# DoHoonKim8/stark-verifier

Measured on AMD Instinct MI355X. Metric: recursive plonky2 proofs/sec (Semaphore d=20), higher is better.
Workload: dtype u64 (Goldilocks field, integer); 1 GPU; recursive: per unit one Semaphore signal (group 2^20, n=2^13, blowup 8, 28 FRI queries, 16 PoW bits, zk) + the recursive proof verifying it (n=2^14, same FRI parameters); 128 units per GPU per step, 10 prover contexts per GPU; all_gather of (nullifier|topic) + Poseidon aggregation root per step; parallelism=independent proofs sharded over ranks, no data-path collective, exchange=none (one rank): gl355_aggregation_root over the local leaves, units_proven_in_process=1674

## Files before the change

### include/gl355.h

```cpp
#ifndef GL355_H
#define GL355_H
#include <stddef.h>
#include <stdint.h>

#ifdef __cplusplus
extern "C" {
#endif

#define GL355_OK 0
#define GL355_E_INVALID_ARG (-1)
#define GL355_E_NO_DEVICE (-2)
#define GL355_E_OOM (-3)
#define GL355_E_HIP (-4)
#define GL355_E_UNSUPPORTED (-5)
#define GL355_E_WITNESS (-6)
#define GL355_E_VERIFY (-7)

#define GL355_P UINT64_C(0xFFFFFFFF00000001)
#define GL355_COSET_SHIFT UINT64_C(7)
#define GL355_SALT_SIZE 4
#define GL355_MAX_FRI_ARITY_BITS 4
#define GL355_MAX_UNITS 16

typedef struct gl355_ctx gl355_ctx;
// ... 354 lines not shown
int32_t gl355_plonk_vk_from_pk(const gl355_plonk_pk* pk, const uint64_t s_g2[16], gl355_plonk_vk** out);
int32_t gl355_plonk_vk_destroy(gl355_plonk_vk* vk);
int32_t gl355_plonk_verify(gl355_ctx* ctx , const gl355_plonk_vk* vk, const uint64_t* instances, const uint32_t* instance_lens,
                           const uint8_t* proof, uint64_t proof_len, int32_t* ok);
int32_t gl355_plonk_verify_batch(gl355_ctx* ctx , const gl355_plonk_vk* vk, uint32_t n_proofs, const uint64_t* instances ,
                                 const uint32_t* instance_lens , const uint8_t* const* proofs, const uint64_t* proof_lens,
                                 const uint8_t seed[32], int32_t* ok, int32_t* first_bad );
const char* gl355_plonk_verify_last_error(void);
int32_t gl355_plonk_verify_stage_ms(double ms[3]);
int32_t gl355_kzg_params_check(gl355_ctx* ctx, const uint64_t* g , uint64_t n_points, const uint64_t* g_lagrange ,
                               uint32_t log_n, const uint64_t s_g2[16], const uint8_t seed[32], int32_t* ok);

int32_t gl355_zs_partial_products(gl355_ctx* ctx, const uint64_t* wires, const uint64_t* sigmas,
                                  const uint64_t* k_is, uint32_t log_n, uint32_t n_routed,
                                  uint32_t max_degree, uint64_t beta, uint64_t gamma,
                                  uint64_t* z_out, uint64_t* pp_out);

enum { GL355_BN_M_MUL = 0, GL355_BN_M_ADD = 1, GL355_BN_M_SUB = 2, GL355_BN_M_CANON = 3, GL355_BN_M_FROM_INT = 4, GL355_BN_M_TO_INT = 5,
       GL355_BN_M_INV = 6, GL355_BN_M_IS_ZERO = 7, GL355_BN_M_EQ = 8, GL355_BN_FQ = 16,
       GL355_BN_F29_MUL = 32, GL355_BN_F29_MUL_FR = 33, GL355_BN_F29_ADD_NORM = 34, GL355_BN_F29_SUB_C2 = 35, GL355_BN_F29_SUB_C4 = 36,
       GL355_BN_F29_SUB_C8 = 37, GL355_BN_F29_SUB_C16 = 38, GL355_BN_F29_NEG_C2 = 39, GL355_BN_F29_FROM_U256 = 40, GL355_BN_F29_TO_U256 = 41,
       GL355_BN_F29_LIFT = 42, GL355_BN_F29_LIFT_INL = 43, GL355_BN_F29_LOWER = 44, GL355_BN_F29_IS_ZERO_MOD = 45, GL355_BN_F29_TABLE_FORM = 46,
       GL355_BN_F29_NORM = 47, GL355_BN_HASH_FR_ENTER = 48, GL355_BN_HASH_FR_LEAVE = 49 };
enum { GL355_BN_CHAIN_XYZZ = 0, GL355_BN_CHAIN_JAC29 = 1, GL355_BN_CHAIN_JAC = 2, GL355_BN_CHAIN_RED29_LIFT = 3, GL355_BN_CHAIN_RED29_RAW = 4,
       GL355_BN_CHAIN_J = 5 };
enum { GL355_BN_STEP_ADD = 0, GL355_BN_STEP_DOUBLE = 1, GL355_BN_STEP_ACC = 2, GL355_BN_STEP_SELF = 3, GL355_BN_STEP_MADD = 4 };
int32_t gl355_bn254_arith_batch(gl355_ctx* ctx, int32_t op, const uint32_t* a , const uint32_t* b , uint32_t* out ,
                                uint64_t n);
int32_t gl355_bn254_g1_chain(gl355_ctx* ctx, int32_t form, const uint32_t* operands , uint32_t n_operands,
                             const uint32_t* steps , uint32_t n_chains, uint32_t n_steps, uint32_t* trace );

enum { GL355_GL_MUL = 0, GL355_GL_MUL_MULTI1 = 1, GL355_GL_MUL_MULTI2 = 2, GL355_GL_MUL_MULTI3 = 3, GL355_GL_MUL_MULTI4 = 4, GL355_GL_MUL_FILL = 5,
       GL355_GL_MUL2_FILL = 6, GL355_GL_SQR = 7, GL355_GL_SBOX = 8, GL355_GL_SBOX4 = 9, GL355_GL_RECOMBINE = 10, GL355_GL_RECOMBINE_MULTI4 = 11,
       GL355_GL_PARTIAL_ROUNDS = 13 };
int32_t gl355_gl_arith_batch(gl355_ctx* ctx, int32_t op, const uint64_t* a , const uint64_t* b , uint64_t* out , uint64_t n);
int32_t gl355_poseidon_permute_lanes(gl355_ctx* ctx, int32_t form, uint64_t* states , uint64_t count);


int32_t gl355_bn254_g1_msm_bits(gl355_ctx* ctx, const uint64_t* points, const gl355_msm_bases* bases , const uint64_t* scalars, uint64_t n,
                                uint32_t n_sets, uint32_t max_bits, uint64_t* results , uint32_t plan_out[4] );
int32_t gl355_plonk_pk_commit_columns(gl355_plonk_pk* pk, uint32_t which, const uint64_t* columns , uint32_t sets, uint64_t tail,
                                      uint64_t* results );

#ifdef __cplusplus
}
#endif
#endif
```

### stark-verifier_amd/csrc/gl_field.cuh

```cuda
#pragma once
#include <hip/hip_runtime.h>
#include <stdint.h>

#define GL_P 0xFFFFFFFF00000001ull
#define GL_EPS 0xFFFFFFFFull

#define GL_DEV __device__ __forceinline__
#define GL_HD __host__ __device__ __forceinline__

#if defined(__HIP_DEVICE_COMPILE__)
#define GL_UNPRED(c) (c)
#else
#define GL_UNPRED(c) __builtin_unpredictable(c)
#endif

GL_HD uint64_t gl_canon(uint64_t a) { return a >= GL_P ? a - GL_P : a; }

GL_HD uint64_t gl_add(uint64_t a, uint64_t b) {
    uint64_t s = a + b;
    if (GL_UNPRED(s < a)) {
        s += GL_EPS;
        if (GL_UNPRED(s < GL_EPS)) s += GL_EPS;
    }
    return s;
}

GL_HD uint64_t gl_add_canonical(uint64_t a, uint64_t c) {
    uint64_t s = a + c;
    if (GL_UNPRED(s < a)) s += GL_EPS;
    return s;
}

GL_HD uint64_t gl_sub(uint64_t a, uint64_t b) {
    uint64_t d = a - b;
    if (GL_UNPRED(a < b)) {
        uint64_t e = d - GL_EPS;
        if (GL_UNPRED(d < GL_EPS)) e -= GL_EPS;
        d = e;
    }
    return d;
}

GL_HD uint64_t gl_neg(uint64_t a) { return gl_sub(0, a); }

#ifndef GL_MUL_VARIANT
#define GL_MUL_VARIANT 1
#endif
#if GL_MUL_VARIANT != 1 && GL_MUL_VARIANT != 2
#error "GL_MUL_VARIANT is 1 (carry steps in inline asm) or 2 (compiler-scheduled)"
#endif
#ifdef GL_EXPERIMENT_NO_HAZARD_NOP
#define GL_HAZARD_NOP ""
#else
#define GL_HAZARD_NOP "s_nop 1\n\t"
#endif
#if defined(__HIPCC__)
#if GL_MUL_VARIANT == 1
GL_DEV uint64_t gl_dev_sub32(uint32_t lo0, uint32_t lo1, uint32_t sub32) {
    uint32_t x0, x1, m;
    asm("v_sub_co_u32_e32 %0, vcc, %3, %5\n\t" GL_HAZARD_NOP ""
        "v_subbrev_co_u32_e32 %1, vcc, 0, %4, vcc\n\t" GL_HAZARD_NOP ""
        "v_cndmask_b32_e64 %2, 0, -1, vcc\n\t"
        "v_sub_co_u32_e32 %0, vcc, %0, %2\n\t" GL_HAZARD_NOP ""
        "v_subbrev_co_u32_e32 %1, vcc, 0, %1, vcc"
        : "=&v"(x0), "=&v"(x1), "=&v"(m) : "v"(lo0), "v"(lo1), "v"(sub32) : "vcc");
    return ((uint64_t)x1 << 32) | x0;
}
GL_DEV uint64_t gl_dev_add_mul_eps(uint64_t x, uint32_t k) {
    uint64_t r, carry;
    uint32_t m;
    asm("v_mad_u64_u32 %0, %1, %3, -1, %4\n\t" GL_HAZARD_NOP "v_cndmask_b32_e64 %2, 0, -1, %1"
        : "=v"(r), "=s"(carry), "=v"(m) : "v"(k), "v"(x));
    return r + (uint64_t)m;
}
GL_DEV uint64_t gl_dev_mid(uint32_t a1, uint32_t b0, uint64_t u, uint32_t* v0) {
    uint64_t v, carry;
    uint32_t ch;
    asm("v_mad_u64_u32 %0, %1, %3, %4, %5\n\t" GL_HAZARD_NOP "v_cndmask_b32_e64 %2, 0, 1, %1"
        : "=v"(v), "=s"(carry), "=v"(ch) : "v"(a1), "v"(b0), "v"(u));
    *v0 = (uint32_t)v;
    return ((uint64_t)ch << 32) | (v >> 32);
}
#else
GL_DEV uint64_t gl_dev_sub32(uint32_t lo0, uint32_t lo1, uint32_t sub32) {
    unsigned long x, y;
    const bool b = __builtin_usubl_overflow(((unsigned long)lo1 << 32) | lo0, (unsigned long)sub32, &x);
    __builtin_usubl_overflow(x, (unsigned long)(b ? 0xFFFFFFFFu : 0u), &y);
    return y;
}
GL_DEV uint64_t gl_dev_add_mul_eps(uint64_t x, uint32_t k) {
    const uint64_t r = (uint64_t)k * 0xFFFFFFFFu + x;
    return r + (r < x ? 0xFFFFFFFFu : 0u);
}
GL_DEV uint64_t gl_dev_mid(uint32_t a1, uint32_t b0, uint64_t u, uint32_t* v0) {
    const uint64_t v = (uint64_t)a1 * b0 + u;
    *v0 = (uint32_t)v;
    return ((uint64_t)(v < u ? 1u : 0u) << 32) | (v >> 32);
}
#endif
#endif

GL_HD uint64_t gl_reduce128(uint64_t lo, uint64_t hi) {
#if defined(__HIP_DEVICE_COMPILE__)
    return gl_dev_add_mul_eps(gl_dev_sub32((uint32_t)lo, (uint32_t)(lo >> 32), (uint32_t)(hi >> 32)), (uint32_t)hi);
#else
    uint32_t hi_hi = (uint32_t)(hi >> 32), hi_lo = (uint32_t)hi;
    uint64_t t0 = lo - hi_hi;
    if (GL_UNPRED(lo < hi_hi)) t0 -= GL_EPS;
    uint64_t t1 = ((uint64_t)hi_lo << 32) - hi_lo;
    uint64_t r = t0 + t1;
    if (GL_UNPRED(r < t1)) r += GL_EPS;
    return r;
#endif
}

GL_HD uint64_t gl_mul(uint64_t a, uint64_t b) {
#if defined(__HIP_DEVICE_COMPILE__)
    const uint32_t a0 = (uint32_t)a, a1 = (uint32_t)(a >> 32), b0 = (uint32_t)b, b1 = (uint32_t)(b >> 32);
    const uint64_t t = (uint64_t)a0 * b0;
    const uint64_t u = (uint64_t)a0 * b1 + (t >> 32);
    uint32_t v0;
    const uint64_t mid = gl_dev_mid(a1, b0, u, &v0);
    const uint64_t w = (uint64_t)a1 * b1 + mid;
    return gl_dev_add_mul_eps(gl_dev_sub32((uint32_t)t, v0, (uint32_t)(w >> 32)), (uint32_t)w);
#else
    unsigned __int128 pr = (unsigned __int128)a * b;
    return gl_reduce128((uint64_t)pr, (uint64_t)(pr >> 64));
#endif
}

GL_HD uint64_t gl_sqr(uint64_t a) { return gl_mul(a, a); }

#if defined(__HIPCC__) && GL_MUL_VARIANT == 1
template <int N>
GL_DEV void gl_mul_multi(const uint64_t (&a)[N], const uint64_t (&b)[N], uint64_t (&r)[N]) {
    static_assert(N >= 1 && N <= 4, "1 .. 4 products");
#define GL_MM_SB() __builtin_amdgcn_sched_barrier(0)
#define GL_MM_READ(INS, ...)                                               \
    do {                                                                   \
        if (N == 1) asm("s_nop 1\n\t" INS : __VA_ARGS__);                  \
        else if (N == 2 && j == 0) asm("s_nop 0\n\t" INS : __VA_ARGS__);   \
        else asm(INS : __VA_ARGS__);                                       \
    } while (0)
    uint32_t a0[N], a1[N], b0[N], b1[N], ch[N], x0[N], x1[N], m[N];
    uint64_t t[N], u[N], v[N], w[N], c[N];
#pragma unroll
    for (int j = 0; j < N; j++) { a0[j] = (uint32_t)a[j]; a1[j] = (uint32_t)(a[j] >> 32); b0[j] = (uint32_t)b[j]; b1[j] = (uint32_t)(b[j] >> 32); }
#pragma unroll
    for (int j = 0; j < N; j++) { t[j] = (uint64_t)a0[j] * b0[j]; u[j] = (uint64_t)a0[j] * b1[j] + (t[j] >> 32); }
    GL_MM_SB();
#pragma unroll
    for (int j = 0; j < N; j++) { asm("v_mad_u64_u32 %0, %1, %2, %3, %4" : "=v"(v[j]), "=s"(c[j]) : "v"(a1[j]), "v"(b0[j]), "v"(u[j])); GL_MM_SB(); }
#pragma unroll
    for (int j = 0; j < N; j++) { GL_MM_READ("v_cndmask_b32_e64 %0, 0, 1, %1", "=v"(ch[j]) : "s"(c[j])); GL_MM_SB(); }
#pragma unroll
    for (int j = 0; j < N; j++) w[j] = (uint64_t)a1[j] * b1[j] + (((uint64_t)ch[j] << 32) | (v[j] >> 32));
    GL_MM_SB();
#pragma unroll
    for (int j = 0; j < N; j++) { asm("v_sub_co_u32_e64 %0, %1, %2, %3" : "=v"(x0[j]), "=s"(c[j]) : "v"((uint32_t)t[j]), "v"((uint32_t)(w[j] >> 32))); GL_MM_SB(); }
#pragma unroll
    for (int j = 0; j < N; j++) { GL_MM_READ("v_subb_co_u32_e64 %0, %1, %2, 0, %1", "=v"(x1[j]), "+s"(c[j]) : "v"((uint32_t)v[j])); GL_MM_SB(); }
#pragma unroll
    for (int j = 0; j < N; j++) { GL_MM_READ("v_cndmask_b32_e64 %0, 0, -1, %1", "=v"(m[j]) : "s"(c[j])); GL_MM_SB(); }
#pragma unroll
    for (int j = 0; j < N; j++) { asm("v_sub_co_u32_e64 %0, %1, %0, %2" : "+v"(x0[j]), "=s"(c[j]) : "v"(m[j])); GL_MM_SB(); }
#pragma unroll
    for (int j = 0; j < N; j++) { GL_MM_READ("v_subb_co_u32_e64 %0, %1, %0, 0, %1", "+v"(x1[j]), "+s"(c[j])); GL_MM_SB(); }
#pragma unroll
    for (int j = 0; j < N; j++) {
        const uint64_t x = ((uint64_t)x1[j] << 32) | x0[j];
        asm("v_mad_u64_u32 %0, %1, %2, -1, %3" : "=v"(r[j]), "=s"(c[j]) : "v"((uint32_t)w[j]), "v"(x));
        GL_MM_SB();
    }
#pragma unroll
    for (int j = 0; j < N; j++) { GL_MM_READ("v_cndmask_b32_e64 %0, 0, 1, %1", "=v"(m[j]) : "s"(c[j])); GL_MM_SB(); }
#pragma unroll
    for (int j = 0; j < N; j++) asm("v_mad_u64_u32 %0, %1, %2, -1, %0" : "+v"(r[j]), "=s"(c[j]) : "v"(m[j]));
#undef GL_MM_READ
#undef GL_MM_SB
}
template <class F>
GL_DEV uint64_t gl_mul_fill(uint64_t a, uint64_t b, F&& fill) {
#define GL_MF_SB() __builtin_amdgcn_sched_barrier(0)
    const uint32_t a0 = (uint32_t)a, a1 = (uint32_t)(a >> 32), b0 = (uint32_t)b, b1 = (uint32_t)(b >> 32);
    const uint64_t t = (uint64_t)a0 * b0;
    const uint64_t u = (uint64_t)a0 * b1 + (t >> 32);
    uint64_t v, c, r;
    uint32_t ch, x0, x1, m;
    GL_MF_SB();
    asm("v_mad_u64_u32 %0, %1, %2, %3, %4" : "=v"(v), "=s"(c) : "v"(a1), "v"(b0), "v"(u)); GL_MF_SB();
    fill(0); GL_MF_SB();
    asm("v_cndmask_b32_e64 %0, 0, 1, %1" : "=v"(ch) : "s"(c)); GL_MF_SB();
    const uint64_t w = (uint64_t)a1 * b1 + (((uint64_t)ch << 32) | (v >> 32)); GL_MF_SB();
    asm("v_sub_co_u32_e64 %0, %1, %2, %3" : "=v"(x0), "=s"(c) : "v"((uint32_t)t), "v"((uint32_t)(w >> 32))); GL_MF_SB();
    fill(1); GL_MF_SB();
    asm("v_subb_co_u32_e64 %0, %1, %2, 0, %1" : "=v"(x1), "+s"(c) : "v"((uint32_t)v)); GL_MF_SB();
    fill(2); GL_MF_SB();
    asm("v_cndmask_b32_e64 %0, 0, -1, %1" : "=v"(m) : "s"(c)); GL_MF_SB();
    asm("v_sub_co_u32_e64 %0, %1, %0, %2" : "+v"(x0), "=s"(c) : "v"(m)); GL_MF_SB();
    fill(3); GL_MF_SB();
    asm("v_subb_co_u32_e64 %0, %1, %0, 0, %1" : "+v"(x1), "+s"(c)); GL_MF_SB();
    const uint64_t x = ((uint64_t)x1 << 32) | x0;
    asm("v_mad_u64_u32 %0, %1, %2, -1, %3" : "=v"(r), "=s"(c) : "v"((uint32_t)w), "v"(x)); GL_MF_SB();
    fill(4); GL_MF_SB();
    asm("v_cndmask_b32_e64 %0, 0, 1, %1" : "=v"(m) : "s"(c)); GL_MF_SB();
    asm("v_mad_u64_u32 %0, %1, %2, -1, %0" : "+v"(r), "=s"(c) : "v"(m));
    return r;
}
template <class F>
GL_DEV void gl_mul2_fill(const uint64_t (&a)[2], const uint64_t (&b)[2], uint64_t (&r)[2], F&& fill) {
// ... 148 lines not shown
```

### stark-verifier_amd/csrc/gl_hook.hip

```cpp
#include "gl355_internal.h"
#include "poseidon_lanes.cuh"

namespace gl355 {

static int hk_gl_width(int32_t op) {
    switch (op) {
    case GL355_GL_MUL: case GL355_GL_MUL_MULTI1: case GL355_GL_MUL_FILL: case GL355_GL_SQR: case GL355_GL_SBOX: case GL355_GL_RECOMBINE: return 1;
    case GL355_GL_MUL_MULTI2: case GL355_GL_MUL2_FILL: return 2;
    case GL355_GL_MUL_MULTI3: return 3;
    case GL355_GL_MUL_MULTI4: case GL355_GL_SBOX4: case GL355_GL_RECOMBINE_MULTI4: return 4;
    case GL355_GL_PARTIAL_ROUNDS: return 12;
    default: return 0;
    }
}

template <int N> GL_DEV void hk_mul_multi(const uint64_t* a, const uint64_t* b, uint64_t* out) {
    uint64_t x[N], y[N], r[N];
#pragma unroll
    for (int j = 0; j < N; j++) { x[j] = a[j]; y[j] = b[j]; }
    gl_mul_multi<N>(x, y, r);
#pragma unroll
    for (int j = 0; j < N; j++) out[j] = r[j];
}

struct HkRow {
    uint64_t xr[5], al, ah;
    GL_DEV HkRow(uint64_t a, uint64_t b) {
#pragma unroll
        for (int k = 0; k < 5; k++) xr[k] = a * (uint64_t)(k + 1) + b;
        al = (uint32_t)b; ah = b >> 32;
    }
    GL_DEV void term(int k) {
        al += (uint64_t)(uint32_t)xr[k] * PSD_CIRC_DEV[k];
        ah += (uint64_t)(uint32_t)(xr[k] >> 32) * PSD_CIRC_DEV[k];
    }
};

__global__ void __launch_bounds__(256) gl_arith_hook_kernel(int32_t op, int32_t width, const uint64_t* a, const uint64_t* b, uint64_t* out, uint64_t n) {
    const uint64_t i = (blockIdx.x * (uint64_t)blockDim.x + threadIdx.x) * (uint64_t)width;
    if (i >= n) return;
    const uint64_t* pa = a + i;
    const uint64_t* pb = b + i;
    uint64_t* po = out + i;
    switch (op) {
// ... 6 lines not shown
        HkRow row(pa[0], pb[0]);
        po[0] = gl_mul_fill(pa[0], pb[0], [&](int k) { row.term(k); });
        po[n] = row.al; po[2 * n] = row.ah;
        break;
    }
    case GL355_GL_MUL2_FILL: {
        HkRow row(pa[0], pb[0]);
        const uint64_t x[2] = {pa[0], pa[1]}, y[2] = {pb[0], pb[1]};
        uint64_t r[2];
        gl_mul2_fill(x, y, r, [&](int k) { row.term(k); });
        po[0] = r[0]; po[1] = r[1];
        po[n] = row.al; po[2 * n] = row.ah;
        po[n + 1] = 0; po[2 * n + 1] = 0;
        break;
    }
    case GL355_GL_SQR: po[0] = gl_sqr(pa[0]); break;
    case GL355_GL_SBOX: po[0] = psd_sbox(pa[0]); break;
    case GL355_GL_SBOX4: {
        uint64_t x0 = pa[0], x1 = pa[1], x2 = pa[2], x3 = pa[3];
        psd_sbox4(x0, x1, x2, x3);
        po[0] = x0; po[1] = x1; po[2] = x2; po[3] = x3;
        break;
    }
    case GL355_GL_RECOMBINE: po[0] = psd_recombine(pa[0], pb[0]); break;
    case GL355_GL_PARTIAL_ROUNDS: {
        uint64_t s[12];
#pragma unroll
        for (int j = 0; j < 12; j++) s[j] = pa[j];
        psd_partial_rounds_b3(s);
#pragma unroll
        for (int j = 0; j < 12; j++) po[j] = s[j];
        break;
    }
    default: {
        const uint64_t al[4] = {pa[0], pa[1], pa[2], pa[3]}, ah[4] = {pb[0], pb[1], pb[2], pb[3]};
        uint64_t r[4];
        psd_recombine_multi<4>(al, ah, r);
        po[0] = r[0]; po[1] = r[1]; po[2] = r[2]; po[3] = r[3];
        break;
    }
    }
}

template <int FORM>
__global__ void __launch_bounds__(64) poseidon_lanes_hook_kernel(uint64_t* states, uint64_t count) {
    __shared__ uint64_t rings[4][24];
    const int li = threadIdx.x & 15, grp = threadIdx.x >> 4;
    uint64_t g = blockIdx.x * 4ull + grp;
    const bool valid = g < count;
    if (!valid) g = 0;
    uint64_t s = (li < 12) ? states[g * 12 + li] : 0;
    s = psd_permute_lanes<FORM>(s, li, rings[grp]);
    if (valid && li < 12) states[g * 12 + li] = gl_canon(s);
}

}

using namespace gl355;

extern "C" {
int32_t gl355_gl_arith_batch(gl355_ctx* h, int32_t op, const uint64_t* a, const uint64_t* b, uint64_t* out, uint64_t n) {
    Ctx* ctx = ctx_of(h);
    if (!ctx) return GL355_E_INVALID_ARG;
    if (hipSetDevice(ctx->device) != hipSuccess) return ctx->fail(GL355_E_HIP, "hipSetDevice failed");
    const int width = hk_gl_width(op);
    if (!width) return ctx->fail(GL355_E_INVALID_ARG, "gl_arith_batch: bad op");
    if (n % (uint64_t)width) return ctx->fail(GL355_E_INVALID_ARG, "gl_arith_batch: n is not a multiple of the op's records per lane");
    if (n == 0) return GL355_OK;
    const bool two = !(op == GL355_GL_SQR || op == GL355_GL_SBOX || op == GL355_GL_SBOX4 || op == GL355_GL_PARTIAL_ROUNDS);
    if (!a || !out || (two && !b)) return ctx->fail(GL355_E_INVALID_ARG, "gl_arith_batch: null argument");
    const uint64_t lanes = n / (uint64_t)width;
    if ((lanes + 255) / 256 > 0x7FFFFFFFull) return ctx->fail(GL355_E_UNSUPPORTED, "gl_arith_batch: too many records");
    const uint64_t out_words = (op == GL355_GL_MUL_FILL || op == GL355_GL_MUL2_FILL) ? 3 * n : n;
    Staged sa(ctx), sb(ctx), so(ctx);
    GL355_TRY(sa.open(a, n * 8, 1));
    GL355_TRY(sb.open(two ? b : a, n * 8, 1));
    GL355_TRY(so.open(out, out_words * 8, 2));
    hipLaunchKernelGGL(gl_arith_hook_kernel, dim3((uint32_t)((lanes + 255) / 256)), dim3(256), 0, ctx->stream, op, (int32_t)width, sa.as<const uint64_t>(),
                       sb.as<const uint64_t>(), so.as<uint64_t>(), n);
    GL355_HIP(ctx, hipGetLastError());
    return so.finish();
}

int32_t gl355_poseidon_permute_lanes(gl355_ctx* h, int32_t form, uint64_t* states, uint64_t count) {
    Ctx* ctx = ctx_of(h);
    if (!ctx) return GL355_E_INVALID_ARG;
    if (hipSetDevice(ctx->device) != hipSuccess) return ctx->fail(GL355_E_HIP, "hipSetDevice failed");
    if (form != 0 && form != 3) return ctx->fail(GL355_E_INVALID_ARG, "poseidon_permute_lanes: form is 0 or 3");
    if (count == 0) return GL355_OK;
    if (!states) return ctx->fail(GL355_E_INVALID_ARG, "poseidon_permute_lanes: null states");
    if ((count + 3) / 4 > 0x7FFFFFFFull) return ctx->fail(GL355_E_UNSUPPORTED, "poseidon_permute_lanes: too many states");
    Staged s(ctx);
    GL355_TRY(s.open(states, count * 96, 3));
    const dim3 grid((uint32_t)((count + 3) / 4)), block(64);
    if (form == 3) hipLaunchKernelGGL(poseidon_lanes_hook_kernel<3>, grid, block, 0, ctx->stream, s.as<uint64_t>(), count);
    else hipLaunchKernelGGL(poseidon_lanes_hook_kernel<0>, grid, block, 0, ctx->stream, s.as<uint64_t>(), count);
    GL355_HIP(ctx, hipGetLastError());
    return s.finish();
}
}
```

### stark-verifier_amd/csrc/poseidon.cuh

```cuda
#pragma once
#include "gl_field.cuh"
#if GL_MUL_VARIANT != 1
#error "poseidon.cuh is written on the inline-asm product and its lock-step groups: GL_MUL_VARIANT 1"
#endif

#define PSD_TABLE_QUAL __device__ __constant__ const
#include "poseidon_tables.h"

namespace gl355 {

GL_DEV uint64_t psd_sbox(uint64_t x) {
    const uint64_t x2 = gl_sqr(x);
    const uint64_t a[2] = {x, x2}, b[2] = {x2, x2};
    uint64_t r[2];
    gl_mul_multi<2>(a, b, r);
    return gl_mul(r[0], r[1]);
}

GL_DEV uint64_t psd_recombine(uint64_t al, uint64_t ah) {
    uint32_t t1 = (uint32_t)(al >> 32), top;
    asm("v_add_co_u32_e32 %0, vcc, %0, %2\n\t" GL_HAZARD_NOP "v_addc_co_u32_e32 %1, vcc, 0, %3, vcc"
        : "+v"(t1), "=v"(top) : "v"((uint32_t)ah), "v"((uint32_t)(ah >> 32)) : "vcc");
    return gl_dev_add_mul_eps(((uint64_t)t1 << 32) | (uint32_t)al, top);
}

GL_DEV void psd_sbox4(uint64_t& x0, uint64_t& x1, uint64_t& x2, uint64_t& x3) {
    const uint64_t a[4] = {x0, x1, x2, x3};
    uint64_t sq[4], c3[4], c4[4], o[4];
    gl_mul_multi<4>(a, a, sq);
    gl_mul_multi<4>(a, sq, c3);
    gl_mul_multi<4>(sq, sq, c4);
    gl_mul_multi<4>(c3, c4, o);
    x0 = o[0]; x1 = o[1]; x2 = o[2]; x3 = o[3];
}
template <int N>
GL_DEV void psd_recombine_multi(const uint64_t (&al)[N], const uint64_t (&ah)[N], uint64_t (&out)[N]) {
    static_assert(N >= 3, "three or more: no wait states of their own");
    uint32_t t1[N], top[N], m[N];
    uint64_t c[N], r[N];
#pragma unroll
    for (int j = 0; j < N; j++) {
        asm("v_add_co_u32_e64 %0, %1, %2, %3" : "=v"(t1[j]), "=s"(c[j]) : "v"((uint32_t)(al[j] >> 32)), "v"((uint32_t)ah[j]));
        __builtin_amdgcn_sched_barrier(0);
    }
#pragma unroll
    for (int j = 0; j < N; j++) {
        asm("v_addc_co_u32_e64 %0, %1, 0, %2, %1" : "=v"(top[j]), "+s"(c[j]) : "v"((uint32_t)(ah[j] >> 32)));
        __builtin_amdgcn_sched_barrier(0);
    }
#pragma unroll
    for (int j = 0; j < N; j++) {
        const uint64_t x = ((uint64_t)t1[j] << 32) | (uint32_t)al[j];
        asm("v_mad_u64_u32 %0, %1, %2, -1, %3" : "=v"(r[j]), "=s"(c[j]) : "v"(top[j]), "v"(x));
        __builtin_amdgcn_sched_barrier(0);
    }
#pragma unroll
    for (int j = 0; j < N; j++) {
        asm("v_cndmask_b32_e64 %0, 0, -1, %1" : "=v"(m[j]) : "s"(c[j]));
        __builtin_amdgcn_sched_barrier(0);
    }
#pragma unroll
    for (int j = 0; j < N; j++) out[j] = r[j] + (uint64_t)m[j];
}

#define PSD_MDS_CHAIN(C0)                                                                                  \
    "v_mad_u64_u32 %0, %1, %2, " #C0 ", %14\n\tv_mad_u64_u32 %0, %1, %3, 15, %0\n\tv_mad_u64_u32 %0, %1, %4, 41, %0\n\t" \
    "v_mad_u64_u32 %0, %1, %5, 16, %0\n\tv_mad_u64_u32 %0, %1, %6, 2, %0\n\tv_mad_u64_u32 %0, %1, %7, 28, %0\n\t"      \
    "v_mad_u64_u32 %0, %1, %8, 13, %0\n\tv_mad_u64_u32 %0, %1, %9, 13, %0\n\tv_mad_u64_u32 %0, %1, %10, 39, %0\n\t"    \
    "v_mad_u64_u32 %0, %1, %11, 18, %0\n\tv_mad_u64_u32 %0, %1, %12, 34, %0\n\tv_mad_u64_u32 %0, %1, %13, 20, %0"
template <int R>
GL_DEV uint64_t psd_mds_chain(const uint32_t (&x)[12], uint64_t addend) {
    uint64_t acc, unused;
#define PSD_X(i) "v"(x[((i) + R) % 12])
    if constexpr (R == 0)
        asm(PSD_MDS_CHAIN(25) : "=&v"(acc), "=&s"(unused) : PSD_X(0), PSD_X(1), PSD_X(2), PSD_X(3), PSD_X(4), PSD_X(5), PSD_X(6),
            PSD_X(7), PSD_X(8), PSD_X(9), PSD_X(10), PSD_X(11), "s"(addend));
    else
        asm(PSD_MDS_CHAIN(17) : "=&v"(acc), "=&s"(unused) : PSD_X(0), PSD_X(1), PSD_X(2), PSD_X(3), PSD_X(4), PSD_X(5), PSD_X(6),
            PSD_X(7), PSD_X(8), PSD_X(9), PSD_X(10), PSD_X(11), "s"(addend));
#undef PSD_X
    return acc;
}
template <int R, class RC>
GL_DEV void psd_mds_rows(uint64_t (&s)[12], const uint32_t (&lo)[12], const uint32_t (&hi)[12], RC rc) {
    if constexpr (R < 12) {
        const uint64_t c0 = rc[R], c1 = rc[R + 1], c2 = rc[R + 2], c3 = rc[R + 3];
        const uint64_t al[4] = {psd_mds_chain<R>(lo, (uint32_t)c0), psd_mds_chain<R + 1>(lo, (uint32_t)c1), psd_mds_chain<R + 2>(lo, (uint32_t)c2),
                                psd_mds_chain<R + 3>(lo, (uint32_t)c3)};
        const uint64_t ah[4] = {psd_mds_chain<R>(hi, c0 >> 32), psd_mds_chain<R + 1>(hi, c1 >> 32), psd_mds_chain<R + 2>(hi, c2 >> 32),
                                psd_mds_chain<R + 3>(hi, c3 >> 32)};
        uint64_t o[4];
        __builtin_amdgcn_sched_barrier(0);
        psd_recombine_multi<4>(al, ah, o);
        s[R] = o[0]; s[R + 1] = o[1]; s[R + 2] = o[2]; s[R + 3] = o[3];
        psd_mds_rows<R + 4, RC>(s, lo, hi, rc);
    }
}
template <class RC>
GL_DEV void psd_mds(uint64_t (&s)[12], RC rc) {
    uint32_t lo[12], hi[12];
#pragma unroll
    for (int i = 0; i < 12; i++) { lo[i] = (uint32_t)s[i]; hi[i] = (uint32_t)(s[i] >> 32); }
    psd_mds_rows<0, RC>(s, lo, hi, rc);
}


#undef PSD_TABLE_QUAL
#define PSD_TABLE_QUAL __device__ __constant__
#include "poseidon_b3tables.h"

typedef const __attribute__((address_space(4))) uint32_t* psd_b3tab;
typedef const __attribute__((address_space(4))) uint64_t* psd_b3add;
GL_DEV void psd_b3_term(uint64_t& lo, uint64_t& hi, uint32_t c, uint64_t v) {
    uint64_t unused;
    asm("v_mad_u64_u32 %0, %2, %3, %4, %0\n\tv_mad_u64_u32 %1, %2, %3, %5, %1"
        : "+v"(lo), "+v"(hi), "=&s"(unused) : "s"(c), "v"((uint32_t)v), "v"((uint32_t)(v >> 32)));
}
GL_DEV void psd_b3_terms5(uint64_t& lo, uint64_t& hi, const uint32_t* c, const uint64_t* v) {
    uint64_t unused;
#define PSD_V(i) "v"((uint32_t)v[i]), "v"((uint32_t)(v[i] >> 32))
    asm("v_mad_u64_u32 %0, %2, %3, %8, %0\n\tv_mad_u64_u32 %1, %2, %3, %9, %1\n\t"
        "v_mad_u64_u32 %0, %2, %4, %10, %0\n\tv_mad_u64_u32 %1, %2, %4, %11, %1\n\t"
        "v_mad_u64_u32 %0, %2, %5, %12, %0\n\tv_mad_u64_u32 %1, %2, %5, %13, %1\n\t"
        "v_mad_u64_u32 %0, %2, %6, %14, %0\n\tv_mad_u64_u32 %1, %2, %6, %15, %1\n\t"
        "v_mad_u64_u32 %0, %2, %7, %16, %0\n\tv_mad_u64_u32 %1, %2, %7, %17, %1"
        : "+v"(lo), "+v"(hi), "=&s"(unused)
        : "s"(c[0]), "s"(c[1]), "s"(c[2]), "s"(c[3]), "s"(c[4]), PSD_V(0), PSD_V(1), PSD_V(2), PSD_V(3), PSD_V(4));
#undef PSD_V
}
GL_DEV void psd_b3_term_first(uint64_t& lo, uint64_t& hi, uint32_t c, uint64_t v, const uint64_t (&add)[2]) {
    uint64_t unused;
    asm("v_mov_b64 %0, %6\n\tv_mov_b64 %1, %7\n\t"
        "v_mad_u64_u32 %0, %2, %3, %4, %0\n\tv_mad_u64_u32 %1, %2, %3, %5, %1"
        : "=&v"(lo), "=&v"(hi), "=&s"(unused) : "s"(c), "v"((uint32_t)v), "v"((uint32_t)(v >> 32)), "s"(add[0]), "s"(add[1]));
}
struct PsdB3Row {
    uint32_t w[14];
    uint64_t a[2];
};
template <int NT>
GL_DEV void psd_b3_load(PsdB3Row& k, psd_b3tab c, psd_b3add add) {
#pragma unroll
    for (int i = 0; i < NT; i++) k.w[i] = c[i];
    k.a[0] = add[0]; k.a[1] = add[1];
}
template <int NX, int NT_NEXT>
GL_DEV void psd_b3_dot(const uint64_t (&u)[12], const uint64_t (&x)[3], PsdB3Row& k, psd_b3tab next, psd_b3add add_next, uint64_t& lo, uint64_t& hi) {
    const PsdB3Row cur = k;
    psd_b3_term_first(lo, hi, cur.w[0], u[1], cur.a);
    __builtin_amdgcn_sched_barrier(0);
    if constexpr (NT_NEXT > 0) psd_b3_load<NT_NEXT>(k, next, add_next);
    __builtin_amdgcn_sched_barrier(0);
    psd_b3_terms5(lo, hi, &cur.w[1], &u[2]);
    psd_b3_terms5(lo, hi, &cur.w[6], &u[7]);
#pragma unroll
    for (int t = 0; t < NX; t++) psd_b3_term(lo, hi, cur.w[11 + t], x[t]);
    __builtin_amdgcn_sched_barrier(0);
}
template <int R>
GL_DEV void psd_b3_out(uint64_t (&o)[12], const uint64_t (&u)[12], const uint64_t (&x)[3], psd_b3tab mac, psd_b3add add, PsdB3Row& k) {
    if constexpr (R < 12) {
        constexpr int W = PSD_B3_ROW_WORDS;
        uint64_t al[4], ah[4], r[4];
        psd_b3_dot<3, 14>(u, x, k, mac + W * (R + 3), add + 2 * (R + 3), al[0], ah[0]);
        psd_b3_dot<3, 14>(u, x, k, mac + W * (R + 4), add + 2 * (R + 4), al[1], ah[1]);
        psd_b3_dot<3, 14>(u, x, k, mac + W * (R + 5), add + 2 * (R + 5), al[2], ah[2]);
        psd_b3_dot<3, (R + 3 < 11 ? 14 : 0)>(u, x, k, mac + W * (R + 6), add + 2 * (R + 6), al[3], ah[3]);
        psd_recombine_multi<4>(al, ah, r);
        o[R] = r[0]; o[R + 1] = r[1]; o[R + 2] = r[2]; o[R + 3] = r[3];
        __builtin_amdgcn_sched_barrier(0);
        psd_b3_out<R + 4>(o, u, x, mac, add, k);
    }
}
GL_DEV void psd_partial_rounds_b3(uint64_t (&s)[12]) {
#pragma unroll 1
    for (int blk = 0; blk < PSD_B3_BLOCKS; blk++) {
        constexpr int W = PSD_B3_ROW_WORDS;
        psd_b3add add = (psd_b3add)PSD_B3_ADD + blk * 2 * 14;
        psd_b3tab mac = (psd_b3tab)PSD_B3_MAC;
        asm volatile("" : "+s"(mac), "+s"(add));
        PsdB3Row k;
        psd_b3_load<12>(k, mac, add);
        __builtin_amdgcn_sched_barrier(0);
        uint64_t x[3], o[12], lo, hi;
        x[0] = psd_sbox(s[0]);
        __builtin_amdgcn_sched_barrier(0);
        psd_b3_dot<1, 13>(s, x, k, mac + W, add + 2, lo, hi);
        x[1] = psd_sbox(psd_recombine(lo, hi));
        __builtin_amdgcn_sched_barrier(0);
        psd_b3_dot<2, 14>(s, x, k, mac + 2 * W, add + 4, lo, hi);
        x[2] = psd_sbox(psd_recombine(lo, hi));
        __builtin_amdgcn_sched_barrier(0);
        psd_b3_out<0>(o, s, x, mac, add, k);
#pragma unroll
        for (int i = 0; i < 12; i++) s[i] = o[i];
    }
    psd_b3add rc26 = (psd_b3add)PSD_ALL_RC + 12 * 26;
    asm volatile("" : "+s"(rc26));
    s[0] = psd_sbox(s[0]);
    psd_mds(s, rc26);
}

constexpr int psd_rounds_per_iter = 2;
GL_DEV void psd_dense_rounds(uint64_t (&s)[12], int r0, int r1) {
#pragma unroll 1
    for (int r = r0; r < r1; r += psd_rounds_per_iter) {
#pragma unroll
        for (int h = 0; h < psd_rounds_per_iter; h++) {
#pragma unroll
            for (int i = 0; i < 12; i += 4) psd_sbox4(s[i], s[i + 1], s[i + 2], s[i + 3]);
            psd_mds(s, &PSD_ALL_RC[12 * (r + h + 1)]);
        }
    }
}
GL_DEV void psd_permute(uint64_t (&s)[12]) {
#pragma unroll
    for (int i = 0; i < 12; i++) s[i] = gl_add_canonical(s[i], PSD_ALL_RC[i]);
    psd_dense_rounds(s, 0, 4);
    psd_partial_rounds_b3(s);
    psd_dense_rounds(s, 26, 30);
}

struct PsdSponge {
    uint64_t s[12];
// ... 8 lines not shown
```

Baseline: 362.0 recursive proofs/s.

## Fold lo/hi carry into hi chain start and shorten Goldilocks reduction tail

The Poseidon MDS and partial-round dot products now seed the high-half accumulation chain with the upper word of the low-half sum. This replaces the separate add/addc recombine step with a single fold (mad by -1 plus a conditional add). The Goldilocks multiply reduction tail is also rewritten to merge the borrow correction into a signed mad, which removes a cndmask/sub pair. Test ops for the row kernels are added to the arith batch hook. The changes are intended to cut VALU instructions per Poseidon round, at the cost of subtler carry reasoning that must hold for the bounded accumulator widths.

```diff
diff --git a/include/gl355.h b/include/gl355.h
--- a/include/gl355.h
+++ b/include/gl355.h
@@ -410,7 +410,7 @@
 
 enum { GL355_GL_MUL = 0, GL355_GL_MUL_MULTI1 = 1, GL355_GL_MUL_MULTI2 = 2, GL355_GL_MUL_MULTI3 = 3, GL355_GL_MUL_MULTI4 = 4, GL355_GL_MUL_FILL = 5,
        GL355_GL_MUL2_FILL = 6, GL355_GL_SQR = 7, GL355_GL_SBOX = 8, GL355_GL_SBOX4 = 9, GL355_GL_RECOMBINE = 10, GL355_GL_RECOMBINE_MULTI4 = 11,
-       GL355_GL_PARTIAL_ROUNDS = 13 };
+       GL355_GL_PARTIAL_ROUNDS = 13, GL355_GL_ROW_DENSE = 14, GL355_GL_ROW_B3 = 15 };
 int32_t gl355_gl_arith_batch(gl355_ctx* ctx, int32_t op, const uint64_t* a , const uint64_t* b , uint64_t* out , uint64_t n);
 int32_t gl355_poseidon_permute_lanes(gl355_ctx* ctx, int32_t form, uint64_t* states , uint64_t count);
 
diff --git a/stark-verifier_amd/csrc/gl_field.cuh b/stark-verifier_amd/csrc/gl_field.cuh
--- a/stark-verifier_amd/csrc/gl_field.cuh
+++ b/stark-verifier_amd/csrc/gl_field.cuh
@@ -56,6 +56,17 @@
 #endif
 #if defined(__HIPCC__)
 #if GL_MUL_VARIANT == 1
+GL_DEV uint64_t gl_dev_reduce_tail(uint32_t lo0, uint32_t lo1, uint32_t w_hi, uint32_t w_lo) {
+    uint32_t x0, x1, d;
+    uint64_t b2, c1, r;
+    asm("v_sub_co_u32_e64 %0, %2, %3, %4\n\t" GL_HAZARD_NOP "v_subb_co_u32_e64 %1, %2, %5, 0, %2"
+        : "=&v"(x0), "=&v"(x1), "=&s"(b2) : "v"(lo0), "v"(w_hi), "v"(lo1));
+    asm("v_mad_u64_u32 %0, %1, %3, -1, %4\n\t" GL_HAZARD_NOP "v_cndmask_b32_e64 %2, 0, 1, %1\n\t"
+        "v_subb_co_u32_e64 %2, %1, %2, 0, %5\n\t"
+        "v_mad_i64_i32 %0, %1, %2, -1, %0"
+        : "=&v"(r), "=&s"(c1), "=&v"(d) : "v"(w_lo), "v"(((uint64_t)x1 << 32) | x0), "s"(b2));
+    return (((uint64_t)((uint32_t)(r >> 32) + d)) << 32) | (uint32_t)r;
+}
 GL_DEV uint64_t gl_dev_sub32(uint32_t lo0, uint32_t lo1, uint32_t sub32) {
     uint32_t x0, x1, m;
     asm("v_sub_co_u32_e32 %0, vcc, %3, %5\n\t" GL_HAZARD_NOP ""
@@ -92,6 +103,9 @@
     const uint64_t r = (uint64_t)k * 0xFFFFFFFFu + x;
     return r + (r < x ? 0xFFFFFFFFu : 0u);
 }
+GL_DEV uint64_t gl_dev_reduce_tail(uint32_t lo0, uint32_t lo1, uint32_t w_hi, uint32_t w_lo) {
+    return gl_dev_add_mul_eps(gl_dev_sub32(lo0, lo1, w_hi), w_lo);
+}
 GL_DEV uint64_t gl_dev_mid(uint32_t a1, uint32_t b0, uint64_t u, uint32_t* v0) {
     const uint64_t v = (uint64_t)a1 * b0 + u;
     *v0 = (uint32_t)v;
@@ -102,7 +116,7 @@
 
 GL_HD uint64_t gl_reduce128(uint64_t lo, uint64_t hi) {
 #if defined(__HIP_DEVICE_COMPILE__)
-    return gl_dev_add_mul_eps(gl_dev_sub32((uint32_t)lo, (uint32_t)(lo >> 32), (uint32_t)(hi >> 32)), (uint32_t)hi);
+    return gl_dev_reduce_tail((uint32_t)lo, (uint32_t)(lo >> 32), (uint32_t)(hi >> 32), (uint32_t)hi);
 #else
     uint32_t hi_hi = (uint32_t)(hi >> 32), hi_lo = (uint32_t)hi;
     uint64_t t0 = lo - hi_hi;
@@ -122,7 +136,7 @@
     uint32_t v0;
     const uint64_t mid = gl_dev_mid(a1, b0, u, &v0);
     const uint64_t w = (uint64_t)a1 * b1 + mid;
-    return gl_dev_add_mul_eps(gl_dev_sub32((uint32_t)t, v0, (uint32_t)(w >> 32)), (uint32_t)w);
+    return gl_dev_reduce_tail((uint32_t)t, v0, (uint32_t)(w >> 32), (uint32_t)w);
 #else
     unsigned __int128 pr = (unsigned __int128)a * b;
     return gl_reduce128((uint64_t)pr, (uint64_t)(pr >> 64));
@@ -143,7 +157,7 @@
         else asm(INS : __VA_ARGS__);                                       \
     } while (0)
     uint32_t a0[N], a1[N], b0[N], b1[N], ch[N], x0[N], x1[N], m[N];
-    uint64_t t[N], u[N], v[N], w[N], c[N];
+    uint64_t t[N], u[N], v[N], w[N], c[N], bw[N];
 #pragma unroll
     for (int j = 0; j < N; j++) { a0[j] = (uint32_t)a[j]; a1[j] = (uint32_t)(a[j] >> 32); b0[j] = (uint32_t)b[j]; b1[j] = (uint32_t)(b[j] >> 32); }
 #pragma unroll
@@ -157,15 +171,9 @@
     for (int j = 0; j < N; j++) w[j] = (uint64_t)a1[j] * b1[j] + (((uint64_t)ch[j] << 32) | (v[j] >> 32));
     GL_MM_SB();
 #pragma unroll
-    for (int j = 0; j < N; j++) { asm("v_sub_co_u32_e64 %0, %1, %2, %3" : "=v"(x0[j]), "=s"(c[j]) : "v"((uint32_t)t[j]), "v"((uint32_t)(w[j] >> 32))); GL_MM_SB(); }
-#pragma unroll
-    for (int j = 0; j < N; j++) { GL_MM_READ("v_subb_co_u32_e64 %0, %1, %2, 0, %1", "=v"(x1[j]), "+s"(c[j]) : "v"((uint32_t)v[j])); GL_MM_SB(); }
-#pragma unroll
-    for (int j = 0; j < N; j++) { GL_MM_READ("v_cndmask_b32_e64 %0, 0, -1, %1", "=v"(m[j]) : "s"(c[j])); GL_MM_SB(); }
-#pragma unroll
-    for (int j = 0; j < N; j++) { asm("v_sub_co_u32_e64 %0, %1, %0, %2" : "+v"(x0[j]), "=s"(c[j]) : "v"(m[j])); GL_MM_SB(); }
-#pragma unroll
-    for (int j = 0; j < N; j++) { GL_MM_READ("v_subb_co_u32_e64 %0, %1, %0, 0, %1", "+v"(x1[j]), "+s"(c[j])); GL_MM_SB(); }
+    for (int j = 0; j < N; j++) { asm("v_sub_co_u32_e64 %0, %1, %2, %3" : "=v"(x0[j]), "=s"(bw[j]) : "v"((uint32_t)t[j]), "v"((uint32_t)(w[j] >> 32))); GL_MM_SB(); }
+#pragma unroll
+    for (int j = 0; j < N; j++) { GL_MM_READ("v_subb_co_u32_e64 %0, %1, %2, 0, %1", "=v"(x1[j]), "+s"(bw[j]) : "v"((uint32_t)v[j])); GL_MM_SB(); }
 #pragma unroll
     for (int j = 0; j < N; j++) {
         const uint64_t x = ((uint64_t)x1[j] << 32) | x0[j];
@@ -175,7 +183,11 @@
 #pragma unroll
     for (int j = 0; j < N; j++) { GL_MM_READ("v_cndmask_b32_e64 %0, 0, 1, %1", "=v"(m[j]) : "s"(c[j])); GL_MM_SB(); }
 #pragma unroll
-    for (int j = 0; j < N; j++) asm("v_mad_u64_u32 %0, %1, %2, -1, %0" : "+v"(r[j]), "=s"(c[j]) : "v"(m[j]));
+    for (int j = 0; j < N; j++) { asm("v_subb_co_u32_e64 %0, %1, %0, 0, %2" : "+v"(m[j]), "+s"(c[j]) : "s"(bw[j])); GL_MM_SB(); }
+#pragma unroll
+    for (int j = 0; j < N; j++) { asm("v_mad_i64_i32 %0, %1, %2, -1, %0" : "+v"(r[j]), "+s"(c[j]) : "v"(m[j])); GL_MM_SB(); }
+#pragma unroll
+    for (int j = 0; j < N; j++) r[j] = ((uint64_t)((uint32_t)(r[j] >> 32) + m[j]) << 32) | (uint32_t)r[j];
 #undef GL_MM_READ
 #undef GL_MM_SB
 }
diff --git a/stark-verifier_amd/csrc/gl_hook.hip b/stark-verifier_amd/csrc/gl_hook.hip
--- a/stark-verifier_amd/csrc/gl_hook.hip
+++ b/stark-verifier_amd/csrc/gl_hook.hip
@@ -2,6 +2,36 @@
 #include "poseidon_lanes.cuh"
 
 namespace gl355 {
+
+template <int N>
+GL_DEV void psd_recombine_multi(const uint64_t (&al)[N], const uint64_t (&ah)[N], uint64_t (&out)[N]) {
+    static_assert(N >= 3, "three or more: no wait states of their own");
+    uint32_t t1[N], top[N], m[N];
+    uint64_t c[N], r[N];
+#pragma unroll
+    for (int j = 0; j < N; j++) {
+        asm("v_add_co_u32_e64 %0, %1, %2, %3" : "=v"(t1[j]), "=s"(c[j]) : "v"((uint32_t)(al[j] >> 32)), "v"((uint32_t)ah[j]));
+        __builtin_amdgcn_sched_barrier(0);
+    }
+#pragma unroll
+    for (int j = 0; j < N; j++) {
+        asm("v_addc_co_u32_e64 %0, %1, 0, %2, %1" : "=v"(top[j]), "+s"(c[j]) : "v"((uint32_t)(ah[j] >> 32)));
+        __builtin_amdgcn_sched_barrier(0);
+    }
+#pragma unroll
+    for (int j = 0; j < N; j++) {
+        const uint64_t x = ((uint64_t)t1[j] << 32) | (uint32_t)al[j];
+        asm("v_mad_u64_u32 %0, %1, %2, -1, %3" : "=v"(r[j]), "=s"(c[j]) : "v"(top[j]), "v"(x));
+        __builtin_amdgcn_sched_barrier(0);
+    }
+#pragma unroll
+    for (int j = 0; j < N; j++) {
+        asm("v_cndmask_b32_e64 %0, 0, -1, %1" : "=v"(m[j]) : "s"(c[j]));
+        __builtin_amdgcn_sched_barrier(0);
+    }
+#pragma unroll
+    for (int j = 0; j < N; j++) out[j] = r[j] + (uint64_t)m[j];
+}
 
 static int hk_gl_width(int32_t op) {
     switch (op) {
@@ -9,7 +39,7 @@
     case GL355_GL_MUL_MULTI2: case GL355_GL_MUL2_FILL: return 2;
     case GL355_GL_MUL_MULTI3: return 3;
     case GL355_GL_MUL_MULTI4: case GL355_GL_SBOX4: case GL355_GL_RECOMBINE_MULTI4: return 4;
-    case GL355_GL_PARTIAL_ROUNDS: return 12;
+    case GL355_GL_PARTIAL_ROUNDS: case GL355_GL_ROW_DENSE: case GL355_GL_ROW_B3: return 12;
     default: return 0;
     }
 }
@@ -82,6 +112,47 @@
         for (int j = 0; j < 12; j++) po[j] = s[j];
         break;
     }
+    case GL355_GL_ROW_DENSE: {
+        uint64_t s[12];
+#pragma unroll
+        for (int j = 0; j < 12; j++) s[j] = pa[j];
+        psd_b3add rc = (psd_b3add)(b + 2);
+        asm volatile("" : "+s"(rc));
+        psd_mds(s, rc);
+#pragma unroll
+        for (int j = 0; j < 12; j++) po[j] = s[j];
+        break;
+    }
+    case GL355_GL_ROW_B3: {
+        uint64_t u[12], x[3], o[12], lo, hi;
+#pragma unroll
+        for (int j = 0; j < 12; j++) { u[j] = pa[j]; o[j] = 0; }
+        x[0] = u[0]; x[1] = u[1]; x[2] = u[2];
+        constexpr int W = PSD_B3_ROW_WORDS;
+        psd_b3add add = (psd_b3add)(b + 2);
+        psd_b3tab mac = (psd_b3tab)PSD_B3_MAC;
+        const uint64_t row = b[0];
+        asm volatile("" : "+s"(mac), "+s"(add));
+        PsdB3Row k;
+        if (row == 0) {
+            psd_b3_load<12>(k, mac, add);
+            __builtin_amdgcn_sched_barrier(0);
+            psd_b3_dot<1, 13>(u, x, k, mac + W, add + 2, lo, hi);
+            o[0] = psd_fold(lo, hi);
+        } else if (row == 1) {
+            psd_b3_load<13>(k, mac + W, add + 2);
+            __builtin_amdgcn_sched_barrier(0);
+            psd_b3_dot<2, 14>(u, x, k, mac + 2 * W, add + 4, lo, hi);
+            o[0] = psd_fold(lo, hi);
+        } else {
+            psd_b3_load<14>(k, mac + 2 * W, add + 4);
+            __builtin_amdgcn_sched_barrier(0);
+            psd_b3_out<0>(o, u, x, mac, add, k);
+        }
+#pragma unroll
+        for (int j = 0; j < 12; j++) po[j] = o[j];
+        break;
+    }
     default: {
         const uint64_t al[4] = {pa[0], pa[1], pa[2], pa[3]}, ah[4] = {pb[0], pb[1], pb[2], pb[3]};
         uint64_t r[4];
@@ -117,6 +188,8 @@
     if (!width) return ctx->fail(GL355_E_INVALID_ARG, "gl_arith_batch: bad op");
     if (n % (uint64_t)width) return ctx->fail(GL355_E_INVALID_ARG, "gl_arith_batch: n is not a multiple of the op's records per lane");
     if (n == 0) return GL355_OK;
+    const bool rows = op == GL355_GL_ROW_DENSE || op == GL355_GL_ROW_B3;
+    if (rows && n < 36) return ctx->fail(GL355_E_INVALID_ARG, "gl_arith_batch: the row ops read 30 words of constants from the head of b: three lanes or more");
     const bool two = !(op == GL355_GL_SQR || op == GL355_GL_SBOX || op == GL355_GL_SBOX4 || op == GL355_GL_PARTIAL_ROUNDS);
     if (!a || !out || (two && !b)) return ctx->fail(GL355_E_INVALID_ARG, "gl_arith_batch: null argument");
     const uint64_t lanes = n / (uint64_t)width;
diff --git a/stark-verifier_amd/csrc/poseidon.cuh b/stark-verifier_amd/csrc/poseidon.cuh
--- a/stark-verifier_amd/csrc/poseidon.cuh
+++ b/stark-verifier_amd/csrc/poseidon.cuh
@@ -33,25 +33,19 @@
     gl_mul_multi<4>(c3, c4, o);
     x0 = o[0]; x1 = o[1]; x2 = o[2]; x3 = o[3];
 }
+GL_DEV uint64_t psd_chain_start(uint64_t al, uint32_t c_hi) { return (uint64_t)((uint32_t)(al >> 32) + c_hi); }
+GL_DEV uint64_t psd_fold(uint64_t al, uint64_t ahp) {
+    return gl_dev_add_mul_eps(((uint64_t)(uint32_t)ahp << 32) | (uint32_t)al, (uint32_t)(ahp >> 32));
+}
 template <int N>
-GL_DEV void psd_recombine_multi(const uint64_t (&al)[N], const uint64_t (&ah)[N], uint64_t (&out)[N]) {
+GL_DEV void psd_fold_multi(const uint64_t (&al)[N], const uint64_t (&ahp)[N], uint64_t (&out)[N]) {
     static_assert(N >= 3, "three or more: no wait states of their own");
-    uint32_t t1[N], top[N], m[N];
+    uint32_t m[N];
     uint64_t c[N], r[N];
 #pragma unroll
     for (int j = 0; j < N; j++) {
-        asm("v_add_co_u32_e64 %0, %1, %2, %3" : "=v"(t1[j]), "=s"(c[j]) : "v"((uint32_t)(al[j] >> 32)), "v"((uint32_t)ah[j]));
-        __builtin_amdgcn_sched_barrier(0);
-    }
-#pragma unroll
-    for (int j = 0; j < N; j++) {
-        asm("v_addc_co_u32_e64 %0, %1, 0, %2, %1" : "=v"(top[j]), "+s"(c[j]) : "v"((uint32_t)(ah[j] >> 32)));
-        __builtin_amdgcn_sched_barrier(0);
-    }
-#pragma unroll
-    for (int j = 0; j < N; j++) {
-        const uint64_t x = ((uint64_t)t1[j] << 32) | (uint32_t)al[j];
-        asm("v_mad_u64_u32 %0, %1, %2, -1, %3" : "=v"(r[j]), "=s"(c[j]) : "v"(top[j]), "v"(x));
+        const uint64_t x = ((uint64_t)(uint32_t)ahp[j] << 32) | (uint32_t)al[j];
+        asm("v_mad_u64_u32 %0, %1, %2, -1, %3" : "=v"(r[j]), "=s"(c[j]) : "v"((uint32_t)(ahp[j] >> 32)), "v"(x));
         __builtin_amdgcn_sched_barrier(0);
     }
 #pragma unroll
@@ -68,16 +62,18 @@
     "v_mad_u64_u32 %0, %1, %5, 16, %0\n\tv_mad_u64_u32 %0, %1, %6, 2, %0\n\tv_mad_u64_u32 %0, %1, %7, 28, %0\n\t"      \
     "v_mad_u64_u32 %0, %1, %8, 13, %0\n\tv_mad_u64_u32 %0, %1, %9, 13, %0\n\tv_mad_u64_u32 %0, %1, %10, 39, %0\n\t"    \
     "v_mad_u64_u32 %0, %1, %11, 18, %0\n\tv_mad_u64_u32 %0, %1, %12, 34, %0\n\tv_mad_u64_u32 %0, %1, %13, 20, %0"
-template <int R>
-GL_DEV uint64_t psd_mds_chain(const uint32_t (&x)[12], uint64_t addend) {
+template <int R, bool VSTART, class A>
+GL_DEV uint64_t psd_mds_chain(const uint32_t (&x)[12], A addend) {
     uint64_t acc, unused;
 #define PSD_X(i) "v"(x[((i) + R) % 12])
-    if constexpr (R == 0)
-        asm(PSD_MDS_CHAIN(25) : "=&v"(acc), "=&s"(unused) : PSD_X(0), PSD_X(1), PSD_X(2), PSD_X(3), PSD_X(4), PSD_X(5), PSD_X(6),
-            PSD_X(7), PSD_X(8), PSD_X(9), PSD_X(10), PSD_X(11), "s"(addend));
-    else
-        asm(PSD_MDS_CHAIN(17) : "=&v"(acc), "=&s"(unused) : PSD_X(0), PSD_X(1), PSD_X(2), PSD_X(3), PSD_X(4), PSD_X(5), PSD_X(6),
-            PSD_X(7), PSD_X(8), PSD_X(9), PSD_X(10), PSD_X(11), "s"(addend));
+#define PSD_MDS_ASM(C0, START)                                                                                                      \
+    asm(PSD_MDS_CHAIN(C0) : "=&v"(acc), "=&s"(unused) : PSD_X(0), PSD_X(1), PSD_X(2), PSD_X(3), PSD_X(4), PSD_X(5), PSD_X(6), PSD_X(7), \
+        PSD_X(8), PSD_X(9), PSD_X(10), PSD_X(11), START((uint64_t)addend))
+    if constexpr (R == 0 && VSTART) PSD_MDS_ASM(25, "v");
+    else if constexpr (R == 0) PSD_MDS_ASM(25, "s");
+    else if constexpr (VSTART) PSD_MDS_ASM(17, "v");
+    else PSD_MDS_ASM(17, "s");
+#undef PSD_MDS_ASM
 #undef PSD_X
     return acc;
 }
@@ -85,13 +81,15 @@
 GL_DEV void psd_mds_rows(uint64_t (&s)[12], const uint32_t (&lo)[12], const uint32_t (&hi)[12], RC rc) {
     if constexpr (R < 12) {
         const uint64_t c0 = rc[R], c1 = rc[R + 1], c2 = rc[R + 2], c3 = rc[R + 3];
-        const uint64_t al[4] = {psd_mds_chain<R>(lo, (uint32_t)c0), psd_mds_chain<R + 1>(lo, (uint32_t)c1), psd_mds_chain<R + 2>(lo, (uint32_t)c2),
-                                psd_mds_chain<R + 3>(lo, (uint32_t)c3)};
-        const uint64_t ah[4] = {psd_mds_chain<R>(hi, c0 >> 32), psd_mds_chain<R + 1>(hi, c1 >> 32), psd_mds_chain<R + 2>(hi, c2 >> 32),
-                                psd_mds_chain<R + 3>(hi, c3 >> 32)};
+        const uint64_t al[4] = {psd_mds_chain<R, false>(lo, (uint32_t)c0), psd_mds_chain<R + 1, false>(lo, (uint32_t)c1),
+                                psd_mds_chain<R + 2, false>(lo, (uint32_t)c2), psd_mds_chain<R + 3, false>(lo, (uint32_t)c3)};
+        const uint64_t ah[4] = {psd_mds_chain<R, true>(hi, psd_chain_start(al[0], (uint32_t)(c0 >> 32))),
+                                psd_mds_chain<R + 1, true>(hi, psd_chain_start(al[1], (uint32_t)(c1 >> 32))),
+                                psd_mds_chain<R + 2, true>(hi, psd_chain_start(al[2], (uint32_t)(c2 >> 32))),
+                                psd_mds_chain<R + 3, true>(hi, psd_chain_start(al[3], (uint32_t)(c3 >> 32)))};
         uint64_t o[4];
         __builtin_amdgcn_sched_barrier(0);
-        psd_recombine_multi<4>(al, ah, o);
+        psd_fold_multi<4>(al, ah, o);
         s[R] = o[0]; s[R + 1] = o[1]; s[R + 2] = o[2]; s[R + 3] = o[3];
         psd_mds_rows<R + 4, RC>(s, lo, hi, rc);
     }
@@ -111,28 +109,38 @@
 
 typedef const __attribute__((address_space(4))) uint32_t* psd_b3tab;
 typedef const __attribute__((address_space(4))) uint64_t* psd_b3add;
-GL_DEV void psd_b3_term(uint64_t& lo, uint64_t& hi, uint32_t c, uint64_t v) {
+#define PSD_MA(C, V) "v_mad_u64_u32 %0, %1, %" #C ", %" #V ", %0"
+#define PSD_C(i) "s"(c[i])
+#define PSD_H(i) "v"(HI ? (uint32_t)(v[i] >> 32) : (uint32_t)v[i])
+template <int K, bool HI>
+GL_DEV void psd_b3_chain(uint64_t& acc, const uint32_t* c, const uint64_t* v) {
+    static_assert(K == 1 || K == 2 || K == 3 || K == 10 || K == 11, "the statement sizes the rows are cut into");
     uint64_t unused;
-    asm("v_mad_u64_u32 %0, %2, %3, %4, %0\n\tv_mad_u64_u32 %1, %2, %3, %5, %1"
-        : "+v"(lo), "+v"(hi), "=&s"(unused) : "s"(c), "v"((uint32_t)v), "v"((uint32_t)(v >> 32)));
-}
-GL_DEV void psd_b3_terms5(uint64_t& lo, uint64_t& hi, const uint32_t* c, const uint64_t* v) {
+    if constexpr (K == 1)
+        asm(PSD_MA(2, 3) : "+v"(acc), "=&s"(unused) : PSD_C(0), PSD_H(0));
+    else if constexpr (K == 2)
+        asm(PSD_MA(2, 4) "\n\t" PSD_MA(3, 5) : "+v"(acc), "=&s"(unused) : PSD_C(0), PSD_C(1), PSD_H(0), PSD_H(1));
+    else if constexpr (K == 3)
+        asm(PSD_MA(2, 5) "\n\t" PSD_MA(3, 6) "\n\t" PSD_MA(4, 7) : "+v"(acc), "=&s"(unused) : PSD_C(0), PSD_C(1), PSD_C(2), PSD_H(0), PSD_H(1), PSD_H(2));
+    else if constexpr (K == 10)
+        asm(PSD_MA(2, 12) "\n\t" PSD_MA(3, 13) "\n\t" PSD_MA(4, 14) "\n\t" PSD_MA(5, 15) "\n\t" PSD_MA(6, 16) "\n\t"
+            PSD_MA(7, 17) "\n\t" PSD_MA(8, 18) "\n\t" PSD_MA(9, 19) "\n\t" PSD_MA(10, 20) "\n\t" PSD_MA(11, 21)
+            : "+v"(acc), "=&s"(unused)
+            : PSD_C(0), PSD_C(1), PSD_C(2), PSD_C(3), PSD_C(4), PSD_C(5), PSD_C(6), PSD_C(7), PSD_C(8), PSD_C(9),
+              PSD_H(0), PSD_H(1), PSD_H(2), PSD_H(3), PSD_H(4), PSD_H(5), PSD_H(6), PSD_H(7), PSD_H(8), PSD_H(9));
+    else
+        asm(PSD_MA(2, 13) "\n\t" PSD_MA(3, 14) "\n\t" PSD_MA(4, 15) "\n\t" PSD_MA(5, 16) "\n\t" PSD_MA(6, 17) "\n\t" PSD_MA(7, 18) "\n\t"
+            PSD_MA(8, 19) "\n\t" PSD_MA(9, 20) "\n\t" PSD_MA(10, 21) "\n\t" PSD_MA(11, 22) "\n\t" PSD_MA(12, 23)
+            : "+v"(acc), "=&s"(unused)
+            : PSD_C(0), PSD_C(1), PSD_C(2), PSD_C(3), PSD_C(4), PSD_C(5), PSD_C(6), PSD_C(7), PSD_C(8), PSD_C(9), PSD_C(10),
+              PSD_H(0), PSD_H(1), PSD_H(2), PSD_H(3), PSD_H(4), PSD_H(5), PSD_H(6), PSD_H(7), PSD_H(8), PSD_H(9), PSD_H(10));
+}
+#undef PSD_H
+#undef PSD_C
+#undef PSD_MA
+GL_DEV void psd_b3_first(uint64_t& lo, uint32_t c, uint64_t v, uint64_t add_lo) {
     uint64_t unused;
-#define PSD_V(i) "v"((uint32_t)v[i]), "v"((uint32_t)(v[i] >> 32))
-    asm("v_mad_u64_u32 %0, %2, %3, %8, %0\n\tv_mad_u64_u32 %1, %2, %3, %9, %1\n\t"
-        "v_mad_u64_u32 %0, %2, %4, %10, %0\n\tv_mad_u64_u32 %1, %2, %4, %11, %1\n\t"
-        "v_mad_u64_u32 %0, %2, %5, %12, %0\n\tv_mad_u64_u32 %1, %2, %5, %13, %1\n\t"
-        "v_mad_u64_u32 %0, %2, %6, %14, %0\n\tv_mad_u64_u32 %1, %2, %6, %15, %1\n\t"
-        "v_mad_u64_u32 %0, %2, %7, %16, %0\n\tv_mad_u64_u32 %1, %2, %7, %17, %1"
-        : "+v"(lo), "+v"(hi), "=&s"(unused)
-        : "s"(c[0]), "s"(c[1]), "s"(c[2]), "s"(c[3]), "s"(c[4]), PSD_V(0), PSD_V(1), PSD_V(2), PSD_V(3), PSD_V(4));
-#undef PSD_V
-}
-GL_DEV void psd_b3_term_first(uint64_t& lo, uint64_t& hi, uint32_t c, uint64_t v, const uint64_t (&add)[2]) {
-    uint64_t unused;
-    asm("v_mov_b64 %0, %6\n\tv_mov_b64 %1, %7\n\t"
-        "v_mad_u64_u32 %0, %2, %3, %4, %0\n\tv_mad_u64_u32 %1, %2, %3, %5, %1"
-        : "=&v"(lo), "=&v"(hi), "=&s"(unused) : "s"(c), "v"((uint32_t)v), "v"((uint32_t)(v >> 32)), "s"(add[0]), "s"(add[1]));
+    asm("v_mov_b64 %0, %4\n\tv_mad_u64_u32 %0, %1, %2, %3, %0" : "=&v"(lo), "=&s"(unused) : "s"(c), "v"((uint32_t)v), "s"(add_lo));
 }
 struct PsdB3Row {
     uint32_t w[14];
@@ -147,14 +155,15 @@
 template <int NX, int NT_NEXT>
 GL_DEV void psd_b3_dot(const uint64_t (&u)[12], const uint64_t (&x)[3], PsdB3Row& k, psd_b3tab next, psd_b3add add_next, uint64_t& lo, uint64_t& hi) {
     const PsdB3Row cur = k;
-    psd_b3_term_first(lo, hi, cur.w[0], u[1], cur.a);
+    psd_b3_first(lo, cur.w[0], u[1], cur.a[0]);
     __builtin_amdgcn_sched_barrier(0);
     if constexpr (NT_NEXT > 0) psd_b3_load<NT_NEXT>(k, next, add_next);
     __builtin_amdgcn_sched_barrier(0);
-    psd_b3_terms5(lo, hi, &cur.w[1], &u[2]);
-    psd_b3_terms5(lo, hi, &cur.w[6], &u[7]);
-#pragma unroll
-    for (int t = 0; t < NX; t++) psd_b3_term(lo, hi, cur.w[11 + t], x[t]);
+    psd_b3_chain<10, false>(lo, &cur.w[1], &u[2]);
+    psd_b3_chain<NX, false>(lo, &cur.w[11], &x[0]);
+    hi = psd_chain_start(lo, (uint32_t)cur.a[1]);
+    psd_b3_chain<11, true>(hi, &cur.w[0], &u[1]);
+    psd_b3_chain<NX, true>(hi, &cur.w[11], &x[0]);
     __builtin_amdgcn_sched_barrier(0);
 }
 template <int R>
@@ -166,7 +175,7 @@
         psd_b3_dot<3, 14>(u, x, k, mac + W * (R + 4), add + 2 * (R + 4), al[1], ah[1]);
         psd_b3_dot<3, 14>(u, x, k, mac + W * (R + 5), add + 2 * (R + 5), al[2], ah[2]);
         psd_b3_dot<3, (R + 3 < 11 ? 14 : 0)>(u, x, k, mac + W * (R + 6), add + 2 * (R + 6), al[3], ah[3]);
-        psd_recombine_multi<4>(al, ah, r);
+        psd_fold_multi<4>(al, ah, r);
         o[R] = r[0]; o[R + 1] = r[1]; o[R + 2] = r[2]; o[R + 3] = r[3];
         __builtin_amdgcn_sched_barrier(0);
         psd_b3_out<R + 4>(o, u, x, mac, add, k);
@@ -186,10 +195,10 @@
         x[0] = psd_sbox(s[0]);
         __builtin_amdgcn_sched_barrier(0);
         psd_b3_dot<1, 13>(s, x, k, mac + W, add + 2, lo, hi);
-        x[1] = psd_sbox(psd_recombine(lo, hi));
+        x[1] = psd_sbox(psd_fold(lo, hi));
         __builtin_amdgcn_sched_barrier(0);
         psd_b3_dot<2, 14>(s, x, k, mac + 2 * W, add + 4, lo, hi);
-        x[2] = psd_sbox(psd_recombine(lo, hi));
+        x[2] = psd_sbox(psd_fold(lo, hi));
         __builtin_amdgcn_sched_barrier(0);
         psd_b3_out<0>(o, s, x, mac, add, k);
 #pragma unroll
```

Result: faster. 377.7 recursive proofs/s, median of 6 (+4.3%).
